# manikya7022/Continual-Learning-for-Dynamic-Video-Quality-Enhancement

Measured on AMD Instinct MI355X. Metric: train frames/sec (2x SR, T=3, 540p->1080p), higher is better.
Workload: dtype bf16

## Files before the change

continual-learning-for-dynamic-video-quality-enhancement_amd/nerve_cl/_engine.py:

```python
from __future__ import annotations

import os
from typing import Dict, Optional

import torch

from . import _nvq as K
from ._nvq import Sl

GROWTH = 32
LAYERS = 5
CORR_LD = 96
BN_EPS = 1e-5
BN_MOM = 0.1

_ws_cache: Dict[torch.device, torch.Tensor] = {}

DEBUG_CAPTURE: Optional[dict] = None

_TAIL_ROWS = int(os.environ.get("NVQ_TAIL_ROWS", "0"))


def _fused_tail_ok(math: int, x: torch.Tensor, Cimg: int, scale: int) -> bool:
    return (math == K.MATH_BF16 and x.dtype == torch.bfloat16 and scale in (2, 3, 4)
# ... 661 lines not shown
            break
        need_dx = f"body.{k}" in dxs
        dd = _new(dev, NI, H, W, F, dtype=act_dtype)
        fused_bwd = (math == K.MATH_BF16 and act_dtype == torch.bfloat16 and F == 64 and sv.pws[k].dtype == torch.bfloat16
                     and sv.dws[k].dtype == torch.bfloat16)
        if bn_sync[k] is not None:
            grp, st = bn_sync[k]
            bsums = _new(dev, T * 2 * F, dtype=torch.float64)
            cnt = K.bn_counts(st, T, F)
            if fused_bwd and os.environ.get("NVQ_FUSED_PW_BWD", "1") != "0":
                K.pw_bn_backward_reduce(dcur, sv.pws[k], B, sv.bn_mean[k], sv.bn_invstd[k], P[pre + "bn.weight"], P[pre + "bn.bias"],
                                        bsums, G.get(pre + "bn.weight"), G.get(pre + "bn.bias"), ws)
                _allreduce_sum_(bsums, grp)
                K.pw_bn_backward_finish(dcur, sv.pws[k], sv.dws[k], B, sv.bn_mean[k], sv.bn_invstd[k], P[pre + "bn.weight"],
                                        P[pre + "bn.bias"], P[pre + "pointwise.weight"], dd, G.get(pre + "pointwise.weight"), bsums,
                                        cnt, ws)
            else:
                dp = _new(dev, NI, H, W, F, dtype=act_dtype)
                K.bn_relu_backward_reduce(dcur, sv.pws[k], B, sv.bn_mean[k], sv.bn_invstd[k], P[pre + "bn.weight"],
                                          P[pre + "bn.bias"], bsums, G.get(pre + "bn.weight"), G.get(pre + "bn.bias"), ws)
                _allreduce_sum_(bsums, grp)
                K.bn_relu_backward_finish(dcur, sv.pws[k], B, sv.bn_mean[k], sv.bn_invstd[k], P[pre + "bn.weight"],
                                          P[pre + "bn.bias"], bsums, cnt, dp)
                _wgrad(Sl(sv.dws[k]), F, Sl(dp), G, pre + "pointwise.weight", None, wq, 1, math=math)
                K.conv_forward(Sl(dp), K.conv_pack(P[pre + "pointwise.weight"], True, F, F, math=math), None, Sl(dd), 1, math=math)
        elif fused_bwd and os.environ.get("NVQ_FUSED_PW_BWD", "1") != "0":
            dgam, dbet = bn_targets if bn_sums is not None else (G.get(pre + "bn.weight"), G.get(pre + "bn.bias"))
            K.pw_bn_backward(dcur, sv.pws[k], sv.dws[k], B, sv.bn_mean[k], sv.bn_invstd[k], P[pre + "bn.weight"],
                             P[pre + "bn.bias"], sv.training, P[pre + "pointwise.weight"], dd, dgam, dbet,
                             G.get(pre + "pointwise.weight"), ws, sums_in=bn_sums)
            bn_sums = None
        else:
            dp = _new(dev, NI, H, W, F, dtype=act_dtype)
            K.bn_relu_backward(dcur, sv.pws[k], B, sv.bn_mean[k], sv.bn_invstd[k], P[pre + "bn.weight"],
                               P[pre + "bn.bias"], sv.training, dp, G.sink(pre + "bn.weight"), G.sink(pre + "bn.bias"), ws)
            _wgrad(Sl(sv.dws[k]), F, Sl(dp), G, pre + "pointwise.weight", None, wq, 1, math=math)
            K.conv_forward(Sl(dp), K.conv_pack(P[pre + "pointwise.weight"], True, F, F, math=math), None, Sl(dd), 1, math=math)
        xin, xin_bn = sv.dw_in[k]
        dww = G.get(pre + "depthwise.weight")
        if fused_bwd and k > 0 and xin.dtype == torch.bfloat16 and os.environ.get("NVQ_FUSED_DW_BWD", "1") != "0":
            if not need_dx and dww is None:
                break
            dx = _new(dev, NI, H, W, F, dtype=act_dtype)
            prev = f"feature_extractor.body.{k - 1}."
            if fuse_sums and sv.training and need_dx and os.environ.get("NVQ_FUSED_PW_BWD", "1") != "0":
                bn_sums = _new(dev, T, 2, F)
                bn_targets = (G.sink(prev + "bn.weight"), G.sink(prev + "bn.bias"))
                K.dwconv_backward(xin, xin_bn, dd, P[pre + "depthwise.weight"], dx, dww, ws,
                                  bn_sums=bn_sums, bn_dgamma=bn_targets[0], bn_dbeta=bn_targets[1])
            else:
                K.dwconv_backward(xin, xin_bn, dd, P[pre + "depthwise.weight"], dx, dww, ws)
            dcur = dx
            continue
        if dww is not None:
            K.dwconv_wgrad(xin, dd, dww, ws, bn=xin_bn)
        if not need_dx:
            break
        if k == 0 and sv.img8 is not None:
            dx = _new(dev, NI, H, W, F, dtype=act_dtype)
            K.dwconv_forward(dd, P[pre + "depthwise.weight"], dx, flip=True, add=dfeat_all, mask=sv.feat0)
        else:
            dx = _new(dev, NI, H, W, F, dtype=act_dtype if k > 0 else torch.float32)
            K.dwconv_forward(dd, P[pre + "depthwise.weight"], dx, flip=True)
        dcur = dx
    if "head" in run:
        hw, hb = G.get("feature_extractor.head.0.weight"), G.get("feature_extractor.head.0.bias")
        if hw is not None or hb is not None:
            hw = hw if hw is not None else torch.empty_like(P["feature_extractor.head.0.weight"])
            if sv.img8 is not None:
                K.conv_wgrad(Sl(sv.img8), g.Cimg, Sl(dcur), hw, hb, ws, 3, math=math)
            else:
                K.head_wgrad(sv.frames, g.slots, dcur, sv.feat0, hw, hb if hb is not None else G.sink("feature_extractor.head.0.bias"),
                             ws, dout2=dfeat_all)
    return dcur, dfeat_all


LIGHT_F = 32
LIGHT_BLOCKS = (2, 3, 4, 5)

def light_forward(P: Dict[str, torch.Tensor], x: torch.Tensor, scale: int, training: bool, math: int = K.MATH_F32,
                  act_dtype: torch.dtype = torch.float32, sync: Optional[dict] = None) -> "tuple[torch.Tensor, Saved]":
    assert act_dtype == torch.float32 or math == K.MATH_BF16
    dev = x.device
    B, Cimg, H, W = x.shape
    F = LIGHT_F
    frames = x.view(B, 1, Cimg, H, W)
    ws = workspace(dev)
    sv = Saved()
    sv.frames, sv.training, sv.math, sv.act_dtype, sv.scale = frames, training, math, act_dtype, scale
    feat0 = _new(dev, B, H, W, F, dtype=act_dtype)
    K.head_forward(frames, [0], P["net.0.weight"], P["net.0.bias"], feat0, math=math)
    sv.feat0, sv.dws, sv.pws, sv.acts, sv.bn_mean, sv.bn_invstd = feat0, [], [], [], [], []
    sv.bn_sync = []
    cur = feat0
    for k in LIGHT_BLOCKS:
        pre = f"net.{k}."
        d = _new(dev, B, H, W, F, dtype=act_dtype)
        K.dwconv_forward(cur, P[pre + "depthwise.weight"], d)
        p = _new(dev, B, H, W, F, dtype=act_dtype)
        K.conv_forward(Sl(d), K.conv_pack(P[pre + "pointwise.weight"], False, F, math=math), None, Sl(p), 1, math=math)
        mean, invstd = _new(dev, 1, F), _new(dev, 1, F)
        grp = sync.get(pre + "bn") if (training and sync) else None
        sv.bn_sync.append(None)
        if grp is not None:
            st = K.new_bn_stats(dev, 1, F)
            K.bn_stats_reduce(p, B, st, ws)
# ... 103 lines not shown
```

continual-learning-for-dynamic-video-quality-enhancement_amd/nerve_cl/_nvq.py:

```python
from __future__ import annotations

import ctypes as C
import os
from typing import Dict, Optional, Sequence

import torch

_HERE = os.path.dirname(os.path.abspath(__file__))
LIB_PATH = os.environ.get("NVQ_LIB", os.path.join(os.path.dirname(_HERE), "libnvq.so"))

MATH_F32 = 0
MATH_BF16 = 1
MAX_T = 8

_lib = None

vp, ci, cl, cf, sz = C.c_void_p, C.c_int, C.c_long, C.c_float, C.c_size_t


class ConvDesc(C.Structure):
    _fields_ = [
        ("inp", vp), ("in_ld", ci), ("in_coff", ci), ("cin", ci),
        ("wpack", vp),
        ("bias", vp),
# ... 37 lines not shown
        ("x_bf16", ci), ("dy_bf16", ci), ("x_plane", C.c_uint), ("variant", ci),
    ]


class WgradReduceJob(C.Structure):
    _fields_ = [
        ("part", vp), ("bias_part", vp), ("dw", vp), ("dbias", vp),
        ("nsplit", ci), ("nci", ci), ("nco", ci), ("taps", ci), ("cout", ci), ("cin_w", ci),
        ("alpha", cf), ("accumulate", ci),
    ]


LAYOUT_MAX_JOBS = 2 * MAX_T + 1
INJECT_MAX_SRC = 4


class GatherJob(C.Structure):
    _fields_ = [("src", vp), ("src_ld", ci), ("src_coff", ci), ("src_bf16", ci), ("dst", vp)]


class InjectJob(C.Structure):
    _fields_ = [("dst", vp), ("dst_ld", ci), ("dst_coff", ci), ("dst_bf16", ci), ("src", vp * INJECT_MAX_SRC)]


_IP = C.POINTER(ci)

SIGNATURES = {
    "nvq_version": (ci, []),
    "nvq_last_error": (C.c_char_p, []),
    "nvq_conv_pack_floats": (sz, [ci, ci, ci, ci]),
    "nvq_conv_pack": (ci, [vp, ci, ci, ci, ci, ci, ci, ci, vp, vp]),
    "nvq_conv_forward": (ci, [C.POINTER(ConvDesc), vp]),
    "nvq_rdb_tail_forward": (ci, [C.POINTER(ConvDesc), C.POINTER(ConvDesc), vp]),
    "nvq_rdb_backward_weights_floats": (sz, [ci]),
    "nvq_rdb_backward_weights": (ci, [vp, vp, vp, vp, vp, vp, ci, vp, vp]),
    "nvq_sizeof_conv_desc": (sz, []),
    "nvq_wgrad_workspace_bytes": (sz, []),
    "nvq_conv_wgrad": (ci, [C.POINTER(WgradDesc), vp]),
    "nvq_conv_wgrad_partial": (ci, [C.POINTER(WgradDesc), C.POINTER(WgradReduceJob), vp]),
    "nvq_wgrad_reduce_batch": (ci, [C.POINTER(WgradReduceJob), ci, vp]),
    "nvq_sizeof_wgrad_desc": (sz, []),
    "nvq_sizeof_wgrad_reduce_job": (sz, []),
    "nvq_conv_pack_batch": (ci, [vp, ci, ci, vp]),
    "nvq_head_forward": (ci, [vp, ci, ci, ci, ci, ci, _IP, ci, vp, vp, ci, vp, ci, ci, vp, ci, vp]),
    "nvq_head_wgrad": (ci, [vp, ci, ci, ci, ci, ci, _IP, ci, vp, ci, vp, ci, vp, ci, ci, vp, vp, vp, sz, ci, ci, vp]),
    "nvq_dwconv_forward": (ci, [vp, ci, vp, ci, vp, ci, ci, ci, ci, ci, ci, ci, vp, vp, vp]),
    "nvq_dwconv_wgrad": (ci, [vp, ci, vp, ci, ci, ci, ci, ci, vp, vp, sz, ci, ci, ci, vp, vp]),
    "nvq_bn_stats": (ci, [vp, ci, ci, ci, ci, ci, ci, cf, cf, _IP, vp, vp, vp, vp, vp, sz, ci, vp]),
    "nvq_bn_eval_stats": (ci, [vp, vp, ci, ci, cf, vp, vp, vp]),
    "nvq_bn_apply_relu": (ci, [vp, ci, ci, ci, ci, ci, ci, vp, vp, vp, vp, vp, ci, vp, ci, ci, ci, vp, ci, ci, ci, ci, ci, vp]),
    "nvq_bn_relu_backward": (ci, [vp, ci, vp, ci, ci, ci, ci, ci, ci, vp, vp, vp, vp, ci, vp, ci, vp, vp, vp, sz, ci, ci, ci, ci, vp]),
    "nvq_dwconv_backward": (ci, [vp, ci, vp, vp, ci, vp, vp, ci, vp, ci, ci, ci, vp, vp, vp, vp, vp, sz, vp]),
    "nvq_dwconv_backward_ex": (ci, [vp, ci, vp, vp, ci, vp, vp, ci, vp, ci, ci, ci, vp, vp, vp, vp, vp, sz, ci, vp]),
    "nvq_dwpw_forward": (ci, [vp, ci, vp, vp, vp, vp, ci, vp, ci, ci, ci, ci, ci, ci, cf, cf, _IP, vp, vp, vp, vp, vp, sz, vp]),
    "nvq_pw_bn_backward": (ci, [vp, ci, ci, vp, ci, vp, ci, ci, ci, ci, ci, vp, vp, vp, vp, ci, vp, vp, ci, vp, vp, vp, vp, vp, sz, vp]),
    "nvq_pw_bn_backward_ex": (ci, [vp, ci, ci, vp, ci, vp, ci, ci, ci, ci, ci, vp, vp, vp, vp, ci, vp, vp, ci, vp, vp, vp, vp, vp, sz, ci,
                                   vp]),
    "nvq_correlation_forward": (ci, [vp, ci, vp, ci, ci, ci, ci, ci, ci, vp, ci, ci, ci, ci, vp]),
    "nvq_correlation_backward": (ci, [ci, vp, ci, vp, ci, ci, ci, ci, ci, ci, vp, ci, ci, ci, ci, ci, ci, ci, vp, ci, vp, vp]),
    "nvq_warp_forward": (ci, [vp, ci, vp, ci, ci, ci, ci, ci, vp, ci, ci, ci, ci, vp]),
    "nvq_warp_backward": (ci, [vp, ci, ci, vp, ci, vp, ci, ci, ci, ci, ci, vp, ci, vp, ci, vp, sz, ci, ci, ci, ci, vp]),
    "nvq_warp_backward_workspace_bytes": (sz, [ci, ci, ci, ci]),
    "nvq_warp_backward_ex": (ci, [vp, ci, ci, vp, ci, vp, ci, ci, ci, ci, ci, vp, ci, vp, ci, vp, sz, ci, ci, ci, ci, ci, vp, sz,
                                  vp]),
    "nvq_tsum_blocks": (ci, [ci, ci]),
    "nvq_tsum_forward": (ci, [vp, ci, vp, ci, ci, ci, ci, ci, ci, vp, ci, vp, ci, vp, ci, ci, vp]),
    "nvq_tsum_backward": (ci, [vp, ci, vp, vp, ci, vp, ci, ci, ci, ci, ci, ci, vp, ci, vp, ci, ci, ci, ci, vp]),
    "nvq_cbam_channel": (ci, [vp, ci, ci, ci, ci, ci, vp, vp, vp, vp, vp, vp]),
    "nvq_cbam_pool": (ci, [vp, ci, vp, ci, ci, ci, ci, vp, vp, ci, vp]),
    "nvq_cbam_spatial_apply": (ci, [vp, ci, vp, vp, vp, ci, ci, ci, ci, vp, vp, ci, ci, ci, ci, vp]),
    "nvq_cbam_bwd_spatial_pre": (ci, [vp, ci, ci, vp, ci, vp, vp, ci, ci, ci, ci, vp, ci, vp]),
    "nvq_cbam_bwd_spatial_conv": (ci, [vp, vp, vp, ci, ci, ci, vp, vp, vp, sz, ci, vp]),
    "nvq_cbam_bwd_spatial_conv_ex": (ci, [vp, vp, vp, ci, ci, ci, vp, vp, vp, sz, ci, ci, vp]),
    "nvq_cbam_bwd_scale": (ci, [vp, ci, ci, vp, ci, vp, vp, vp, vp, ci, ci, ci, ci, vp, ci, vp, ci, vp]),
    "nvq_cbam_bwd_channel": (ci, [vp, ci, ci, ci, ci, ci, vp, vp, vp, vp, vp, vp, vp, vp, ci, vp]),
    "nvq_cbam_bwd_channel_ex": (ci, [vp, ci, ci, ci, ci, ci, vp, vp, vp, vp, vp, vp, vp, vp, ci, ci, vp]),
    "nvq_upsampler_tail_forward": (ci, [C.POINTER(ConvDesc), vp, ci, ci, ci, ci, vp, vp, vp]),
    "nvq_shuffle_bicubic_clamp": (ci, [vp, ci, vp, ci, ci, ci, ci, ci, ci, ci, vp, vp, vp]),
    "nvq_shuffle_clamp_backward": (ci, [vp, vp, ci, ci, ci, ci, ci, vp, ci, vp]),
    "nvq_bicubic_blend": (ci, [vp, vp, ci, ci, ci, ci, ci, ci, ci, cf, vp, vp]),
    "nvq_head_dgrad": (ci, [vp, ci, ci, vp, ci, vp, ci, ci, vp, ci, ci, ci, ci, ci, ci, _IP, ci, vp, ci, vp]),
    "nvq_bicubic_adjoint": (ci, [vp, vp, ci, ci, ci, ci, ci, ci, ci, cf, vp, ci, vp]),
    "nvq_head_dgrad_tc": (ci, [vp, ci, ci, vp, ci, ci, ci, ci, ci, ci, _IP, _IP, ci, ci, vp, ci, vp]),
    "nvq_stem7_dgrad": (ci, [vp, ci, ci, vp, ci, ci, ci, ci, vp, vp, ci, vp]),
    "nvq_mask_blend_backward_ex": (ci, [vp, vp, vp, ci, vp, ci, ci, ci, ci, vp, vp, vp, vp]),
    "nvq_nchw_to_nhwc": (ci, [vp, cl, ci, ci, ci, ci, vp, ci, ci, ci, vp]),
    "nvq_nhwc_to_nchw": (ci, [vp, ci, ci, ci, ci, ci, ci, vp, cl, vp]),
    "nvq_gather_nchw": (ci, [vp, ci, ci, ci, ci, ci, vp]),
    "nvq_inject_nchw": (ci, [vp, ci, ci, ci, ci, ci, vp]),
    "nvq_sizeof_gather_job": (sz, []),
    "nvq_sizeof_inject_job": (sz, []),
    "nvq_bn2_workspace_bytes": (sz, [ci]),
    "nvq_bn2_stats": (ci, [vp, ci, ci, cl, cf, cf, vp, vp, vp, vp, vp, sz, ci, vp]),
    "nvq_bn2_eval_stats": (ci, [vp, vp, ci, cf, vp, vp, vp]),
    "nvq_bn2_apply": (ci, [vp, ci, ci, cl, vp, vp, vp, vp, vp, ci, ci, vp, ci, ci, vp]),
    "nvq_bn2_backward": (ci, [vp, ci, vp, ci, ci, cl, vp, vp, vp, vp, vp, ci, ci, ci, vp, ci, vp, ci, vp, vp, vp, sz, ci, vp]),
    "nvq_bn2_backward_ex": (ci, [vp, ci, vp, ci, ci, cl, vp, vp, vp, vp, vp, ci, ci, ci, vp, ci, vp, ci, vp, vp, vp, sz, ci, ci, vp]),
    "nvq_bn_stats_reduce": (ci, [vp, ci, ci, ci, ci, ci, ci, vp, vp, sz, ci, vp]),
    "nvq_bn_stats_finish": (ci, [vp, ci, ci, cf, cf, _IP, vp, vp, vp, vp, vp]),
    "nvq_dwpw_forward_sums": (ci, [vp, ci, vp, vp, vp, vp, ci, vp, ci, ci, ci, ci, ci, vp, vp, sz, vp]),
    "nvq_bn_relu_backward_reduce": (ci, [vp, ci, vp, ci, ci, ci, ci, ci, ci, vp, vp, vp, vp, vp, vp, vp, vp, sz, ci, ci, ci, vp]),
    "nvq_bn_relu_backward_finish": (ci, [vp, ci, vp, ci, ci, ci, ci, ci, ci, vp, vp, vp, vp, vp, vp, vp, ci, ci, ci, ci, vp]),
    "nvq_pw_bn_backward_reduce": (ci, [vp, ci, ci, vp, ci, ci, ci, ci, ci, vp, vp, vp, vp, vp, vp, vp, vp, sz, vp]),
    "nvq_pw_bn_backward_finish": (ci, [vp, ci, ci, vp, ci, vp, ci, ci, ci, ci, ci, vp, vp, vp, vp, vp, vp, ci, vp, vp, vp, vp, sz,
                                       ci, vp]),
    "nvq_bn2_stats_reduce": (ci, [vp, ci, ci, cl, vp, vp, sz, ci, vp]),
# ... 527 lines not shown
    check(lib().nvq_bn_stats(ptr(x), ld, Cc, N, group_images, H, W, eps, momentum, int_array(order), ptr(mean),
                             ptr(invstd), ptr(rmean), ptr(rvar), ptr(ws), ws.numel() * 4, is_bf16(x), stream()),
          "nvq_bn_stats")


def bn_eval_stats(rmean, rvar, G: int, mean, invstd, eps=1e-5):
    check(lib().nvq_bn_eval_stats(ptr(rmean), ptr(rvar), rmean.numel(), G, eps, ptr(mean), ptr(invstd), stream()),
          "nvq_bn_eval_stats")


def bn_apply_relu(x: torch.Tensor, group_images: int, mean, invstd, gamma, beta, res: Optional[torch.Tensor],
                  outA: Sl, split_images: int, outB: Optional[Sl] = None):
    N, H, W, ld = x.shape
    Cc = gamma.numel()
    check(lib().nvq_bn_apply_relu(ptr(x), ld, Cc, N, group_images, H, W, ptr(mean), ptr(invstd), ptr(gamma),
                                  ptr(beta), ptr(res), res.shape[-1] if res is not None else 0, ptr(outA.t),
                                  outA.ld, outA.coff, split_images, ptr(outB.t) if outB else None,
                                  outB.ld if outB else 0, outB.coff if outB else 0, is_bf16(x), outA.bf16, is_bf16(res),
                                  stream()),
          "nvq_bn_apply_relu")


def bn_relu_backward(dy: torch.Tensor, x: torch.Tensor, group_images: int, mean, invstd, gamma, beta,
                     training: bool, dx: torch.Tensor, dgamma, dbeta, ws, accumulate=False):
    N, H, W, ld = x.shape
    Cc = gamma.numel()
    check(lib().nvq_bn_relu_backward(ptr(dy), dy.shape[-1], ptr(x), ld, Cc, N, group_images, H, W, ptr(mean),
                                     ptr(invstd), ptr(gamma), ptr(beta), int(training), ptr(dx), dx.shape[-1],
                                     ptr(dgamma), ptr(dbeta), ptr(ws), ws.numel() * 4, int(accumulate), is_bf16(dy),
                                     is_bf16(x), is_bf16(dx), stream()),
          "nvq_bn_relu_backward")


def dwconv_backward(x: torch.Tensor, bn, dy: torch.Tensor, weight: torch.Tensor, dx: torch.Tensor, dweight, ws,
                    add: Optional[torch.Tensor] = None, mask: Optional[torch.Tensor] = None, bn_sums=None, bn_dgamma=None,
                    bn_dbeta=None) -> None:
    N, H, W, ld = x.shape
    assert x.dtype == dy.dtype == dx.dtype == torch.bfloat16 and weight.shape[0] == 64
    b = _bn_input(bn)
    e = None
    if add is not None or mask is not None:
        e = DwEpilogue()
        e.add, e.add_ld, e.add_bf16 = ptr(add), add.shape[-1] if add is not None else 0, is_bf16(add)
        e.mask, e.mask_ld, e.mask_bf16 = ptr(mask), mask.shape[-1] if mask is not None else 0, is_bf16(mask)
    args = (ptr(x), ld, C.byref(b) if b is not None else None, ptr(dy), dy.shape[-1], ptr(weight.contiguous()), ptr(dx),
            dx.shape[-1], C.byref(e) if e is not None else None, N, H, W, ptr(dweight), ptr(bn_sums), ptr(bn_dgamma),
            ptr(bn_dbeta), ptr(ws), ws.numel() * 4)
    if dweight is None:
        check(lib().nvq_dwconv_backward_ex(*args, NO_WGRAD, stream()), "nvq_dwconv_backward_ex")
        return
    check(lib().nvq_dwconv_backward(*args, stream()), "nvq_dwconv_backward")


def dwpw_forward(x: torch.Tensor, bn, dw_weight: torch.Tensor, pw_weight: torch.Tensor, d: torch.Tensor, p: torch.Tensor,
                 group_images: int, order: Optional[Sequence[int]], mean, invstd, rmean, rvar, ws, eps=1e-5,
                 momentum=0.1) -> None:
    N, H, W, ld = x.shape
    assert x.dtype == d.dtype == p.dtype == torch.bfloat16 and tuple(pw_weight.shape[:2]) == (64, 64)
    b = _bn_input(bn)
    stats = order is not None
    ev0 = TIMER.start() if TIMER is not None else None
    check(lib().nvq_dwpw_forward(ptr(x), ld, C.byref(b) if b is not None else None, ptr(dw_weight.contiguous()),
                                 ptr(pw_weight.contiguous()), ptr(d), d.shape[-1], ptr(p), p.shape[-1], N, group_images, H, W,
                                 int(stats), eps, momentum, int_array(order) if stats else None, ptr(mean) if stats else None,
                                 ptr(invstd) if stats else None, ptr(rmean) if stats else None, ptr(rvar) if stats else None,
                                 ptr(ws), ws.numel() * 4, stream()), "nvq_dwpw_forward")
    if ev0 is not None:
        npx = N * H * W
        TIMER.stop(ev0, "dwpw_fwd_kernel", 2.0 * npx * 64 * (64 + 9), npx * 64 * 2.0 * 3, f"n{N} 64->64")


def pw_bn_backward(dy: torch.Tensor, p: torch.Tensor, d: torch.Tensor, group_images: int, mean, invstd, gamma, beta,
                   training: bool, weight: torch.Tensor, dd: torch.Tensor, dgamma, dbeta, dweight, ws, sums_in=None) -> None:
    N, H, W, _ = p.shape
    assert p.dtype == d.dtype == dd.dtype == torch.bfloat16 and tuple(weight.shape[:2]) == (64, 64)
    ev0 = TIMER.start() if TIMER is not None else None
    args = (ptr(dy), dy.shape[-1], is_bf16(dy), ptr(p), p.shape[-1], ptr(d), d.shape[-1], N, group_images, H, W, ptr(mean),
            ptr(invstd), ptr(gamma), ptr(beta), int(training), ptr(weight.contiguous()), ptr(dd), dd.shape[-1], ptr(dgamma),
            ptr(dbeta), ptr(dweight), ptr(sums_in), ptr(ws), ws.numel() * 4)
    if dweight is None or dgamma is None or dbeta is None:
        check(lib().nvq_pw_bn_backward_ex(*args, NO_WGRAD if dweight is None else 0, stream()), "nvq_pw_bn_backward_ex")
    else:
        check(lib().nvq_pw_bn_backward(*args, stream()), "nvq_pw_bn_backward")
    if ev0 is not None:
        npx = N * H * W
        TIMER.stop(ev0, "pw_bn_bwd_kernel", 2.0 * npx * 64 * 64 * 2,
                   npx * 64 * (2.0 * 2 + (2 if is_bf16(dy) else 4) * 2 + 2), f"n{N} 64->64 {'h' if is_bf16(dy) else 'f'}")


def new_bn_stats(dev, G: int, Cc: int) -> torch.Tensor:
    return torch.empty(G * 2 * Cc + G, dtype=torch.float64, device=dev)


def bn_counts(stats: torch.Tensor, G: int, Cc: int) -> torch.Tensor:
    return stats[G * 2 * Cc:]


def bn_stats_reduce(x: torch.Tensor, group_images: int, stats: torch.Tensor, ws) -> None:
    N, H, W, ld = x.shape
    Cc = (stats.numel() // (N // group_images) - 1) // 2
    check(lib().nvq_bn_stats_reduce(ptr(x), ld, Cc, N, group_images, H, W, ptr(stats), ptr(ws), ws.numel() * 4, is_bf16(x),
                                    stream()), "nvq_bn_stats_reduce")


def bn_stats_finish(stats: torch.Tensor, G: int, order: Sequence[int], mean, invstd, rmean, rvar, eps=1e-5,
                    momentum=0.1) -> None:
# ... 608 lines not shown
```

include/nvq.h:

```cpp
#ifndef NVQ_H
#define NVQ_H

#include <stddef.h>
#include <stdint.h>

#ifdef __cplusplus
extern "C" {
#endif

#define NVQ_OK 0
#define NVQ_EINVAL (-1)
#define NVQ_ELAUNCH (-2)
#define NVQ_EWORKSPACE (-3)

#define NVQ_MATH_F32 0
#define NVQ_MATH_BF16 1

#define NVQ_MAX_T 8

int nvq_version(void);
const char* nvq_last_error(void);


size_t nvq_conv_pack_floats(int cout, int cin_store, int ksize, int math);
// ... 55 lines not shown
    int nsplit, nci, nco, taps, cout, cin_w; float alpha; int accumulate;
} nvq_wgrad_reduce_job;
int nvq_conv_wgrad_partial(const nvq_wgrad_desc* d, nvq_wgrad_reduce_job* job, void* stream);
int nvq_wgrad_reduce_batch(const nvq_wgrad_reduce_job* jobs, int n, void* stream);
size_t nvq_sizeof_wgrad_desc(void);
size_t nvq_sizeof_wgrad_reduce_job(void);

int nvq_pw_bn_backward(const float* dy, int dy_ld, int dy_bf16, const float* p, int p_ld, const float* d, int d_ld,
                       int N, int group_images, int H, int W, const float* mean, const float* invstd,
                       const float* gamma, const float* beta, int training, const float* weight, float* dd, int dd_ld,
                       float* dgamma, float* dbeta, float* dweight, const float* sums_in, float* workspace,
                       size_t workspace_bytes, void* stream);
#define NVQ_NO_WGRAD 2
int nvq_pw_bn_backward_ex(const float* dy, int dy_ld, int dy_bf16, const float* p, int p_ld, const float* d, int d_ld,
                          int N, int group_images, int H, int W, const float* mean, const float* invstd,
                          const float* gamma, const float* beta, int training, const float* weight, float* dd, int dd_ld,
                          float* dgamma, float* dbeta, float* dweight, const float* sums_in, float* workspace,
                          size_t workspace_bytes, int flags, void* stream);

int nvq_head_forward(const float* frames, int B, int T, int Cin, int H, int W,
                     const int* t_of_slot_host, int nslots,
                     const float* weight, const float* bias, int F,
                     float* out, int out_ld, int out_bf16, float* img8, int math, void* stream);
int nvq_head_wgrad(const float* frames, int B, int T, int Cin, int H, int W,
                   const int* t_of_slot_host, int nslots,
                   const float* dout, int dout_ld, const float* dout2, int dout2_ld,
                   const float* act, int act_ld, int F,
                   float* dweight, float* dbias, float* workspace, size_t workspace_bytes,
                   int accumulate, int act_bf16, void* stream);

typedef struct nvq_bn_input {
    const float* mean; const float* invstd; const float* gamma; const float* beta;
    int group_images;
} nvq_bn_input;
typedef struct nvq_dw_epilogue {
    const float* add; int add_ld; const float* mask; int mask_ld; int mask_bf16; int add_bf16;
} nvq_dw_epilogue;
int nvq_dwconv_forward(const float* in, int in_ld, const float* weight, int C,
                       float* out, int out_ld, int N, int H, int W, int flip,
                       int in_bf16, int out_bf16, const nvq_bn_input* bn, const nvq_dw_epilogue* epi,
                       void* stream);
int nvq_dwconv_wgrad(const float* x, int x_ld, const float* dy, int dy_ld, int C,
                     int N, int H, int W, float* dweight, float* workspace,
                     size_t workspace_bytes, int accumulate, int x_bf16, int dy_bf16,
                     const nvq_bn_input* bn, void* stream);
int nvq_dwconv_backward(const float* x, int x_ld, const nvq_bn_input* bn, const float* dy, int dy_ld, const float* weight,
                        float* dx, int dx_ld, const nvq_dw_epilogue* epi, int N, int H, int W, float* dweight,
                        float* bn_sums, float* bn_dgamma, float* bn_dbeta, float* workspace, size_t workspace_bytes,
                        void* stream);
int nvq_dwconv_backward_ex(const float* x, int x_ld, const nvq_bn_input* bn, const float* dy, int dy_ld, const float* weight,
                           float* dx, int dx_ld, const nvq_dw_epilogue* epi, int N, int H, int W, float* dweight,
                           float* bn_sums, float* bn_dgamma, float* bn_dbeta, float* workspace, size_t workspace_bytes,
                           int flags, void* stream);
int nvq_dwpw_forward(const float* in, int in_ld, const nvq_bn_input* bn, const float* dw_weight, const float* pw_weight,
                     float* d, int d_ld, float* p, int p_ld, int N, int group_images, int H, int W, int stats, float eps,
                     float momentum, const int* order_host, float* mean, float* invstd, float* running_mean, float* running_var,
                     float* workspace, size_t workspace_bytes, void* stream);

int nvq_bn_stats(const float* x, int x_ld, int C, int N, int group_images, int H, int W,
                 float eps, float momentum, const int* order_host,
                 float* mean, float* invstd, float* running_mean, float* running_var,
                 float* workspace, size_t workspace_bytes, int x_bf16, void* stream);
int nvq_bn_eval_stats(const float* running_mean, const float* running_var, int C, int G,
                      float eps, float* mean, float* invstd, void* stream);
int nvq_bn_apply_relu(const float* x, int x_ld, int C, int N, int group_images, int H, int W,
                      const float* mean, const float* invstd, const float* gamma,
                      const float* beta, const float* res, int res_ld,
                      float* outA, int outA_ld, int outA_coff, int split_images,
                      float* outB, int outB_ld, int outB_coff, int x_bf16, int out_bf16, int res_bf16,
                      void* stream);
int nvq_bn_relu_backward(const float* dy, int dy_ld, const float* x, int x_ld, int C, int N,
                         int group_images, int H, int W, const float* mean, const float* invstd,
                         const float* gamma, const float* beta, int training,
                         float* dx, int dx_ld, float* dgamma, float* dbeta,
                         float* workspace, size_t workspace_bytes, int accumulate,
                         int dy_bf16, int x_bf16, int dx_bf16, void* stream);

int nvq_correlation_forward(const float* x1, int x1_ld, const float* x2, int x2_ld,
                            int x2_images, int C, int N, int H, int W,
                            float* out, int out_ld, int math, int out_bf16, int in_bf16, void* stream);
typedef struct nvq_corr_addends {
    const void* a; int a_ld; int a_coff;
    const void* b; int b_ld; int b_coff;
} nvq_corr_addends;
int nvq_correlation_backward(int which, const float* dcorr, int dcorr_ld,
                             const float* other, int other_ld, int other_images, int C, int N,
                             int H, int W, float* dx, int dx_ld, int dx_coff, int accumulate,
                             int math, int dcorr_bf16, int other_bf16, int groups, float* dx_bf16_out, int dx_bf16_ld,
                             const nvq_corr_addends* addends, void* stream);

int nvq_warp_forward(const float* feat, int feat_ld, const float* flow, int flow_ld,
                     int C, int N, int H, int W, float* out, int out_ld, int out_coff,
                     int feat_bf16, int out_bf16, void* stream);
int nvq_warp_backward(const float* dout, int dout_ld, int dout_coff, const float* feat,
                      int feat_ld, const float* flow, int flow_ld, int C, int N, int H, int W,
                      float* dfeat, int dfeat_ld, float* dflow, int dflow_ld,
                      float* records, size_t records_bytes, int feat_bf16, int dout_bf16, int overwrite, int dfeat_bf16,
                      void* stream);
#define NVQ_WARP_DETERMINISTIC 1
size_t nvq_warp_backward_workspace_bytes(int N, int H, int W, int flags);
int nvq_warp_backward_ex(const float* dout, int dout_ld, int dout_coff, const float* feat,
                         int feat_ld, const float* flow, int flow_ld, int C, int N, int H, int W,
                         float* dfeat, int dfeat_ld, float* dflow, int dflow_ld,
                         float* records, size_t records_bytes, int feat_bf16, int dout_bf16, int overwrite,
                         int dfeat_bf16, int flags, void* workspace, size_t workspace_bytes, void* stream);

// ... 288 lines not shown
```

Before: 78.66.

## Fuse first-layer depthwise backward with head conv weight/bias gradients

Adds a HIP kernel that, for the first feature-extractor layer, computes the depthwise weight gradient, applies the flipped depthwise conv plus skip add and ReLU mask to form the head's output gradient in LDS, and then reduces the head conv weight and bias gradients with MFMA, all in one tiled pass. This replaces separate dwconv_wgrad, dwconv_forward, and head conv_wgrad launches, which each re-read the large 64-channel activations from memory. When frame gradients are needed it still runs a separate dwconv_forward for dx. The cost is a complex kernel with per-workgroup partials and extra reductions, and a bf16 rounding of the intermediate gradient.

```diff
diff --git a/continual-learning-for-dynamic-video-quality-enhancement_amd/csrc/head_bwd.hip b/continual-learning-for-dynamic-video-quality-enhancement_amd/csrc/head_bwd.hip
--- /dev/null
+++ b/continual-learning-for-dynamic-video-quality-enhancement_amd/csrc/head_bwd.hip
@@ -0,0 +1,297 @@
+#include "conv_common.h"
+
+namespace nvq {
+namespace {
+
+typedef unsigned u32x4 __attribute__((ext_vector_type(4)));
+typedef unsigned u32x2 __attribute__((ext_vector_type(2)));
+typedef short s16x4 __attribute__((ext_vector_type(4)));
+typedef s16x4 __attribute__((address_space(3))) * lds_s16x4_ptr;
+
+constexpr int FH = 8, FW = 32, FHW = FW + 2, FNPIX = (FH + 2) * FHW;
+constexpr int FC = 64;
+constexpr int FT = 256;
+constexpr int PER = (FNPIX * 8 + FT - 1) / FT;
+constexpr int XPER = FH * FW * 8 / FT;
+static_assert(PER * FT - FNPIX * 8 >= FNPIX - FT, "the frame pixels beyond the first FT ride in the last dd piece");
+constexpr int IW = FHW + 2;
+constexpr int IC = 4;
+constexpr int FMAXWG = 512;
+constexpr int RU = 5;
+constexpr int NHW = FC * 27;
+
+struct HeadBwdArgs {
+    const __bf16* x; int x_ld;
+    const __bf16* dd; int dd_ld;
+    const __bf16* add; int add_ld;
+    const __bf16* img; int img_ld;
+    const float* w;
+    float *part_dw, *part_hw, *part_hb;
+    int H, W, tilesX, tilesY, ntiles;
+};
+
+__device__ __forceinline__ float4 unpack4(u32x2 v) {
+    return make_float4(__uint_as_float(v[0] << 16), __uint_as_float(v[0] & 0xffff0000u), __uint_as_float(v[1] << 16),
+                       __uint_as_float(v[1] & 0xffff0000u));
+}
+
+template <bool WG>
+__global__ __launch_bounds__(FT, 2) void head_bwd_kernel(const HeadBwdArgs a) {
+    __shared__ __attribute__((aligned(16))) __bf16 gs[FNPIX * FC];
+    __shared__ __attribute__((aligned(16))) __bf16 xs[FH * FW * FC];
+    __shared__ __attribute__((aligned(16))) __bf16 is[(FH + 2) * IW * IC];
+    const int tid = threadIdx.x;
+    const int wave = __builtin_amdgcn_readfirstlane(tid >> 6), lane = tid & 63;
+
+    for (int i = tid; i < (FH + 2) * IW * IC / 2; i += FT) reinterpret_cast<unsigned*>(is)[i] = 0u;
+    const int c4 = tid & 15, xcol = tid >> 4;
+    float4 wf[9], wacc[9];
+#pragma unroll
+    for (int t = 0; t < 9; ++t) {
+        const int c = 4 * c4, tt = 8 - t;
+        wf[t] = make_float4(a.w[(c + 0) * 9 + tt], a.w[(c + 1) * 9 + tt], a.w[(c + 2) * 9 + tt], a.w[(c + 3) * 9 + tt]);
+        wacc[t] = make_float4(0.f, 0.f, 0.f, 0.f);
+    }
+    f32x4 hacc[3];
+#pragma unroll
+    for (int ky = 0; ky < 3; ++ky) hacc[ky] = (f32x4){0.f, 0.f, 0.f, 0.f};
+
+    const int tiles_per_image = a.tilesX * a.tilesY;
+    u32x4 v[PER], xv[XPER];
+    u32x2 iv;
+    unsigned okm = 0;
+    constexpr int XB = PER, IB = PER + XPER;
+    auto locate = [&](int t, int& n, int& ty, int& tx) {
+        int bt = xcd_tile(t, a.ntiles);
+        n = bt / tiles_per_image;
+        bt -= n * tiles_per_image;
+        ty = bt / a.tilesX;
+        tx = bt - ty * a.tilesX;
+    };
+    auto fetch = [&](int t) {
+        int n, ty, tx;
+        locate(t, n, ty, tx);
+        okm = 0;
+        int tid_o = tid;
+        asm volatile("" : "+v"(tid_o));
+#pragma unroll
+        for (int k = 0; k < PER; ++k) {
+            const int item = tid_o + k * FT;
+            const bool isimg = k == PER - 1 && item >= FNPIX * 8;
+            const int hp = isimg ? item - FNPIX * 8 + FT : item >> 3, q = item & 7;
+            const int hy = hp / FHW, hx = hp - hy * FHW;
+            const int gy = ty * FH + hy - 1, gx = tx * FW + hx - 1;
+            const bool ok = hp < FNPIX && gy >= 0 && gy < a.H && gx >= 0 && gx < a.W;
+            okm |= (ok ? 1u : 0u) << k;
+            const size_t pix = ok ? (size_t)(n * a.H + gy) * a.W + gx : 0;
+            v[k] = *reinterpret_cast<const u32x4*>(isimg ? a.img + pix * a.img_ld : a.dd + pix * a.dd_ld + (ok ? 8 * q : 0));
+        }
+#pragma unroll
+        for (int k = 0; k < XPER; ++k) {
+            const int item = tid_o + k * FT;
+            const int px = item >> 3, q = item & 7;
+            const int gy = ty * FH + (px >> 5), gx = tx * FW + (px & 31);
+            const bool ok = gy < a.H && gx < a.W;
+            okm |= (ok ? 1u : 0u) << (XB + k);
+            xv[k] = *reinterpret_cast<const u32x4*>(a.x + (ok ? ((size_t)(n * a.H + gy) * a.W + gx) * a.x_ld + 8 * q : 0));
+        }
+    };
+    auto fetch_img = [&](int t) {
+        int n, ty, tx;
+        locate(t, n, ty, tx);
+        int tid_o = tid;
+        asm volatile("" : "+v"(tid_o));
+        const int hy = tid_o / FHW, hx = tid_o - hy * FHW;
+        const int gy = ty * FH + hy - 1, gx = tx * FW + hx - 1;
+        const bool ok = gy >= 0 && gy < a.H && gx >= 0 && gx < a.W;
+        okm |= (ok ? 1u : 0u) << IB;
+        iv = *reinterpret_cast<const u32x2*>(a.img + (ok ? ((size_t)(n * a.H + gy) * a.W + gx) * a.img_ld : 0));
+    };
+    auto commit_img = [&](int hp, unsigned lo, unsigned hi, bool ok) {
+        const int hy = hp / FHW, hx = hp - hy * FHW;
+        const u32x2 o = {ok ? lo : 0u, (ok ? hi & 0xffffu : 0u) | 0x3f800000u};
+        *reinterpret_cast<u32x2*>(is + (hy * IW + hx) * IC) = o;
+    };
+    auto commit = [&]() {
+        int tid_c = tid;
+        asm volatile("" : "+v"(tid_c));
+#pragma unroll
+        for (int k = 0; k < PER; ++k) {
+            const int item = tid_c + k * FT;
+            u32x4 o;
+#pragma unroll
+            for (int e = 0; e < 4; ++e) o[e] = (okm >> k) & 1 ? v[k][e] : 0u;
+            if (item < FNPIX * 8) *reinterpret_cast<u32x4*>(gs + (item >> 3) * FC + 8 * (item & 7)) = o;
+            else if (item - FNPIX * 8 + FT < FNPIX) commit_img(item - FNPIX * 8 + FT, o[0], o[1], true);
+            asm volatile("" ::: "memory");
+        }
+#pragma unroll
+        for (int k = 0; k < XPER; ++k) {
+            const int item = tid_c + k * FT;
+            u32x4 o;
+#pragma unroll
+            for (int e = 0; e < 4; ++e) o[e] = (okm >> (XB + k)) & 1 ? xv[k][e] : 0u;
+            *reinterpret_cast<u32x4*>(xs + (item >> 3) * FC + 8 * (item & 7)) = o;
+            asm volatile("" ::: "memory");
+        }
+        commit_img(tid_c, iv[0], iv[1], (okm >> IB) & 1);
+    };
+
+    int t = blockIdx.x;
+    if (t < a.ntiles) { fetch(t); fetch_img(t); }
+    __syncthreads();
+    for (; t < a.ntiles; t += gridDim.x) {
+        int n, ty, tx;
+        locate(t, n, ty, tx);
+        commit();
+        __syncthreads();
+        if (t + (int)gridDim.x < a.ntiles) fetch(t + gridDim.x);
+
+        const float4 z4 = make_float4(0.f, 0.f, 0.f, 0.f);
+#pragma unroll 1
+        for (int h = 0; h < 2; ++h) {
+            const int x = xcol + 16 * h;
+            const int gx = tx * FW + x;
+            float4 a0 = z4, a1 = z4, a2 = z4;
+            float4 X0 = z4, X1 = z4, X2 = z4;
+#pragma unroll 1
+            for (int r0 = 0; r0 < FH + 2; r0 += RU)
+#pragma unroll
+            for (int ri = 0; ri < RU; ++ri) {
+                const int rr = r0 + ri;
+                if (rr < FH) X0 = unpack4(*reinterpret_cast<const u32x2*>(xs + (rr * FW + x) * FC + 4 * c4));
+#pragma unroll
+                for (int b = 0; b < 3; ++b) {
+                    const float4 vv = unpack4(*reinterpret_cast<const u32x2*>(gs + (rr * FHW + x + b) * FC + 4 * c4));
+                    if (rr < FH) {
+                        const float4 ww = wf[b]; float4& s = wacc[b];
+                        a0.x = __builtin_fmaf(vv.x, ww.x, a0.x); a0.y = __builtin_fmaf(vv.y, ww.y, a0.y); a0.z = __builtin_fmaf(vv.z, ww.z, a0.z); a0.w = __builtin_fmaf(vv.w, ww.w, a0.w);
+                        if constexpr (WG) { s.x += vv.x * X0.x; s.y += vv.y * X0.y; s.z += vv.z * X0.z; s.w += vv.w * X0.w; }
+                    }
+                    if (rr >= 1 && rr <= FH) {
+                        const float4 ww = wf[3 + b]; float4& s = wacc[3 + b];
+                        a1.x = __builtin_fmaf(vv.x, ww.x, a1.x); a1.y = __builtin_fmaf(vv.y, ww.y, a1.y); a1.z = __builtin_fmaf(vv.z, ww.z, a1.z); a1.w = __builtin_fmaf(vv.w, ww.w, a1.w);
+                        if constexpr (WG) { s.x += vv.x * X1.x; s.y += vv.y * X1.y; s.z += vv.z * X1.z; s.w += vv.w * X1.w; }
+                    }
+                    if (rr >= 2) {
+                        const float4 ww = wf[6 + b]; float4& s = wacc[6 + b];
+                        a2.x = __builtin_fmaf(vv.x, ww.x, a2.x); a2.y = __builtin_fmaf(vv.y, ww.y, a2.y); a2.z = __builtin_fmaf(vv.z, ww.z, a2.z); a2.w = __builtin_fmaf(vv.w, ww.w, a2.w);
+                        if constexpr (WG) { s.x += vv.x * X2.x; s.y += vv.y * X2.y; s.z += vv.z * X2.z; s.w += vv.w * X2.w; }
+                    }
+                }
+                if (rr >= 2) {
+                    const int gy = ty * FH + rr - 2;
+                    float4 o = a2;
+                    if (gy < a.H && gx < a.W) {
+                        const size_t pix = (size_t)(n * a.H + gy) * a.W + gx;
+                        const float4 ad = unpack4(*reinterpret_cast<const u32x2*>(a.add + pix * a.add_ld + 4 * c4));
+                        o.x += ad.x; o.y += ad.y; o.z += ad.z; o.w += ad.w;
+                    }
+                    if (!(X2.x > 0.f)) o.x = 0.f;
+                    if (!(X2.y > 0.f)) o.y = 0.f;
+                    if (!(X2.z > 0.f)) o.z = 0.f;
+                    if (!(X2.w > 0.f)) o.w = 0.f;
+                    const bf16x4 ob = {(__bf16)o.x, (__bf16)o.y, (__bf16)o.z, (__bf16)o.w};
+                    *reinterpret_cast<bf16x4*>(xs + ((rr - 2) * FW + x) * FC + 4 * c4) = ob;
+                }
+                a2 = a1; a1 = a0; a0 = z4;
+                X2 = X1; X1 = X0; X0 = z4;
+            }
+        }
+        __syncthreads();
+        if (t + (int)gridDim.x < a.ntiles) fetch_img(t + gridDim.x);
+
+        int lane_o = lane;
+        asm volatile("" : "+v"(lane_o));
+        const int trg = lane_o >> 4, trq = (lane_o >> 2) & 3, trp = lane_o & 3;
+        const __bf16* abase = xs + (4 * trg + trq) * FC + wave * 16 + 4 * trp;
+        const __bf16* bbase = is + (4 * trg + trq + trp) * IC;
+#pragma unroll 1
+        for (int r = 0; r < FH; ++r) {
+            const s16x4 al = __builtin_amdgcn_ds_read_tr16_b64_v4i16((lds_s16x4_ptr)(abase + r * FW * FC));
+            const s16x4 ah = __builtin_amdgcn_ds_read_tr16_b64_v4i16((lds_s16x4_ptr)(abase + r * FW * FC + 16 * FC));
+            const bf16x8 af = __builtin_bit_cast(bf16x8, __builtin_shufflevector(al, ah, 0, 1, 2, 3, 4, 5, 6, 7));
+#pragma unroll
+            for (int ky = 0; ky < 3; ++ky) {
+                const s16x4 bl = __builtin_amdgcn_ds_read_tr16_b64_v4i16((lds_s16x4_ptr)(bbase + (r + ky) * IW * IC));
+                const s16x4 bh = __builtin_amdgcn_ds_read_tr16_b64_v4i16((lds_s16x4_ptr)(bbase + (r + ky) * IW * IC + 16 * IC));
+                const bf16x8 bf = __builtin_bit_cast(bf16x8, __builtin_shufflevector(bl, bh, 0, 1, 2, 3, 4, 5, 6, 7));
+                hacc[ky] = __builtin_amdgcn_mfma_f32_16x16x32_bf16(af, bf, hacc[ky], 0, 0, 0);
+            }
+        }
+        __syncthreads();
+    }
+
+    {
+        float* prow = a.part_hw + (size_t)blockIdx.x * NHW;
+        const int kx = (lane & 15) >> 2, ci = lane & 3;
+        if (kx < 3 && ci < 3)
+#pragma unroll
+            for (int ky = 0; ky < 3; ++ky)
+#pragma unroll
+                for (int r = 0; r < 4; ++r) prow[(16 * wave + 4 * (lane >> 4) + r) * 27 + ci * 9 + ky * 3 + kx] = hacc[ky][r];
+    }
+    if ((lane & 15) == 7)
+#pragma unroll
+        for (int r = 0; r < 4; ++r) a.part_hb[(size_t)blockIdx.x * FC + 16 * wave + 4 * (lane >> 4) + r] = hacc[1][r];
+    if constexpr (WG) {
+        float* red = reinterpret_cast<float*>(gs);
+#pragma unroll
+        for (int t9 = 0; t9 < 9; ++t9) {
+            float s[4] = {wacc[t9].x, wacc[t9].y, wacc[t9].z, wacc[t9].w};
+#pragma unroll
+            for (int e = 0; e < 4; ++e) {
+                s[e] += __shfl_xor(s[e], 16, 64);
+                s[e] += __shfl_xor(s[e], 32, 64);
+                if (lane < 16) red[(wave * 16 + lane) * 36 + (8 - t9) * 4 + e] = s[e];
+            }
+        }
+        __syncthreads();
+        float* prow = a.part_dw + (size_t)blockIdx.x * FC * 9;
+        for (int i = tid; i < 16 * 36; i += FT) {
+            const int ci = i / 36, k = i - ci * 36;
+            const float s = red[(0 * 16 + ci) * 36 + k] + red[(1 * 16 + ci) * 36 + k] + red[(2 * 16 + ci) * 36 + k] +
+                            red[(3 * 16 + ci) * 36 + k];
+            prow[(4 * ci + (k & 3)) * 9 + (k >> 2)] = s;
+        }
+    }
+}
+
+}
+}
+
+using namespace nvq;
+
+extern "C" int nvq_first_layer_backward(const float* feat0, int feat0_ld, const float* dd, int dd_ld, const float* dfeat,
+                                        int dfeat_ld, const float* img8, int img8_ld, const float* dw_weight, int N, int H,
+                                        int W, float* d_dw_weight, float* d_head_weight, float* d_head_bias, float* workspace,
+                                        size_t workspace_bytes, void* stream) {
+    NVQ_REQUIRE(feat0 && dd && dfeat && img8 && dw_weight && N > 0 && H > 0 && W > 0, "first_layer_backward: operands");
+    NVQ_REQUIRE(d_dw_weight || d_head_weight || d_head_bias, "first_layer_backward: no gradient is wanted");
+    NVQ_REQUIRE(feat0_ld % 8 == 0 && dd_ld % 8 == 0 && feat0_ld >= FC && dd_ld >= FC && aligned16(feat0) && aligned16(dd),
+                "first_layer_backward: 64-channel bf16 tensors, 16-byte addressable");
+    NVQ_REQUIRE(dfeat_ld % 4 == 0 && dfeat_ld >= FC && aligned8(dfeat), "first_layer_backward: dfeat (bf16, 8-byte addressable)");
+    NVQ_REQUIRE(img8_ld % 8 == 0 && img8_ld >= 8 && aligned16(img8), "first_layer_backward: img8 (bf16, 16-byte addressable)");
+    NVQ_REQUIRE((long)N * H * W < ((long)1 << 31), "first_layer_backward: too many pixels");
+    const int tilesX = (W + FW - 1) / FW, tilesY = (H + FH - 1) / FH;
+    const int ntiles = tilesX * tilesY * N;
+    int nwg = ntiles < FMAXWG ? ntiles : FMAXWG;
+    if (nwg >= 8) nwg &= ~7;
+    const size_t dw_floats = (size_t)nwg * FC * 9, hw_floats = (size_t)nwg * NHW, hb_floats = (size_t)nwg * FC;
+    if ((dw_floats + hw_floats + hb_floats) * sizeof(float) > workspace_bytes) {
+        set_error("first_layer_backward: workspace");
+        return NVQ_EWORKSPACE;
+    }
+    HeadBwdArgs a{reinterpret_cast<const __bf16*>(feat0), feat0_ld, reinterpret_cast<const __bf16*>(dd), dd_ld,
+                  reinterpret_cast<const __bf16*>(dfeat), dfeat_ld, reinterpret_cast<const __bf16*>(img8), img8_ld, dw_weight,
+                  workspace, workspace + dw_floats, workspace + dw_floats + hw_floats, H, W, tilesX, tilesY, ntiles};
+    hipStream_t s = (hipStream_t)stream;
+    if (d_dw_weight) hipLaunchKernelGGL(head_bwd_kernel<true>, dim3(nwg), dim3(FT), 0, s, a);
+    else hipLaunchKernelGGL(head_bwd_kernel<false>, dim3(nwg), dim3(FT), 0, s, a);
+    int rc = check_launch("first_layer_backward");
+    if (rc) return rc;
+    if (d_dw_weight) rc = launch_reduce_partials(a.part_dw, nwg, FC * 9, 1.f, d_dw_weight, 0, s);
+    if (!rc && d_head_weight) rc = launch_reduce_partials(a.part_hw, nwg, NHW, 1.f, d_head_weight, 0, s);
+    if (!rc && d_head_bias) rc = launch_reduce_partials(a.part_hb, nwg, FC, 1.f, d_head_bias, 0, s);
+    return rc;
+}
diff --git a/continual-learning-for-dynamic-video-quality-enhancement_amd/nerve_cl/_engine.py b/continual-learning-for-dynamic-video-quality-enhancement_amd/nerve_cl/_engine.py
--- a/continual-learning-for-dynamic-video-quality-enhancement_amd/nerve_cl/_engine.py
+++ b/continual-learning-for-dynamic-video-quality-enhancement_amd/nerve_cl/_engine.py
@@ -737,6 +737,16 @@
                 K.dwconv_backward(xin, xin_bn, dd, P[pre + "depthwise.weight"], dx, dww, ws)
             dcur = dx
             continue
+        if (k == 0 and fused_bwd and sv.img8 is not None and g.Cimg == 3 and xin is sv.feat0 and xin_bn is None
+                and dfeat_all.dtype == torch.bfloat16 and os.environ.get("NVQ_FUSED_HEAD_BWD", "1") != "0"):
+            hw, hb = G.get("feature_extractor.head.0.weight"), G.get("feature_extractor.head.0.bias")
+            if dww is not None or hw is not None or hb is not None:
+                K.first_layer_backward(sv.feat0, dd, dfeat_all, sv.img8, P[pre + "depthwise.weight"], dww, hw, hb, ws)
+            if not plan.frames:
+                return None, dfeat_all
+            dx = _new(dev, NI, H, W, F, dtype=act_dtype)
+            K.dwconv_forward(dd, P[pre + "depthwise.weight"], dx, flip=True, add=dfeat_all, mask=sv.feat0)
+            return dx, dfeat_all
         if dww is not None:
             K.dwconv_wgrad(xin, dd, dww, ws, bn=xin_bn)
         if not need_dx:
diff --git a/continual-learning-for-dynamic-video-quality-enhancement_amd/nerve_cl/_nvq.py b/continual-learning-for-dynamic-video-quality-enhancement_amd/nerve_cl/_nvq.py
--- a/continual-learning-for-dynamic-video-quality-enhancement_amd/nerve_cl/_nvq.py
+++ b/continual-learning-for-dynamic-video-quality-enhancement_amd/nerve_cl/_nvq.py
@@ -113,6 +113,7 @@
     "nvq_bn_relu_backward": (ci, [vp, ci, vp, ci, ci, ci, ci, ci, ci, vp, vp, vp, vp, ci, vp, ci, vp, vp, vp, sz, ci, ci, ci, ci, vp]),
     "nvq_dwconv_backward": (ci, [vp, ci, vp, vp, ci, vp, vp, ci, vp, ci, ci, ci, vp, vp, vp, vp, vp, sz, vp]),
     "nvq_dwconv_backward_ex": (ci, [vp, ci, vp, vp, ci, vp, vp, ci, vp, ci, ci, ci, vp, vp, vp, vp, vp, sz, ci, vp]),
+    "nvq_first_layer_backward": (ci, [vp, ci, vp, ci, vp, ci, vp, ci, vp, ci, ci, ci, vp, vp, vp, vp, sz, vp]),
     "nvq_dwpw_forward": (ci, [vp, ci, vp, vp, vp, vp, ci, vp, ci, ci, ci, ci, ci, ci, cf, cf, _IP, vp, vp, vp, vp, vp, sz, vp]),
     "nvq_pw_bn_backward": (ci, [vp, ci, ci, vp, ci, vp, ci, ci, ci, ci, ci, vp, vp, vp, vp, ci, vp, vp, ci, vp, vp, vp, vp, vp, sz, vp]),
     "nvq_pw_bn_backward_ex": (ci, [vp, ci, ci, vp, ci, vp, ci, ci, ci, ci, ci, vp, vp, vp, vp, ci, vp, vp, ci, vp, vp, vp, vp, vp, sz, ci,
@@ -746,6 +747,17 @@
     check(lib().nvq_dwconv_backward(*args, stream()), "nvq_dwconv_backward")
 
 
+def first_layer_backward(feat0: torch.Tensor, dd: torch.Tensor, dfeat: torch.Tensor, img8: torch.Tensor, weight: torch.Tensor,
+                         dweight, dhead_weight, dhead_bias, ws) -> None:
+    N, H, W, ld = feat0.shape
+    assert feat0.dtype == dd.dtype == dfeat.dtype == img8.dtype == torch.bfloat16 and weight.shape[0] == 64
+    assert tuple(dd.shape[:3]) == tuple(dfeat.shape[:3]) == tuple(img8.shape[:3]) == (N, H, W)
+    assert dhead_weight is None or tuple(dhead_weight.shape) == (64, 3, 3, 3)
+    check(lib().nvq_first_layer_backward(ptr(feat0), ld, ptr(dd), dd.shape[-1], ptr(dfeat), dfeat.shape[-1], ptr(img8),
+                                         img8.shape[-1], ptr(weight.contiguous()), N, H, W, ptr(dweight), ptr(dhead_weight),
+                                         ptr(dhead_bias), ptr(ws), ws.numel() * 4, stream()), "nvq_first_layer_backward")
+
+
 def dwpw_forward(x: torch.Tensor, bn, dw_weight: torch.Tensor, pw_weight: torch.Tensor, d: torch.Tensor, p: torch.Tensor,
                  group_images: int, order: Optional[Sequence[int]], mean, invstd, rmean, rvar, ws, eps=1e-5,
                  momentum=0.1) -> None:
diff --git a/include/nvq.h b/include/nvq.h
--- a/include/nvq.h
+++ b/include/nvq.h
@@ -131,6 +131,10 @@
                            float* dx, int dx_ld, const nvq_dw_epilogue* epi, int N, int H, int W, float* dweight,
                            float* bn_sums, float* bn_dgamma, float* bn_dbeta, float* workspace, size_t workspace_bytes,
                            int flags, void* stream);
+int nvq_first_layer_backward(const float* feat0, int feat0_ld, const float* dd, int dd_ld, const float* dfeat, int dfeat_ld,
+                             const float* img8, int img8_ld, const float* dw_weight, int N, int H, int W,
+                             float* d_dw_weight, float* d_head_weight, float* d_head_bias, float* workspace,
+                             size_t workspace_bytes, void* stream);
 int nvq_dwpw_forward(const float* in, int in_ld, const nvq_bn_input* bn, const float* dw_weight, const float* pw_weight,
                      float* d, int d_ld, float* p, int p_ld, int N, int group_images, int H, int W, int stats, float eps,
                      float momentum, const int* order_host, float* mean, float* invstd, float* running_mean, float* running_var,
```

Result: no change. 79.15 (median of 6 runs) (+0.6%).
